# UWQuickstep/quickstep

Measured on AMD Instinct MI355X. Metric: probe+aggregate rows/s at TPC-H SF100 (Q1,Q3), higher is better.
Workload: dtype i32 keys / f64 sums

## Files before the change

quickstep_amd/csrc/join.hip:

```cpp

#include "common.hpp"
#include "join_dense.hpp"
#include "join_lds.hpp"
#include "scan.hpp"

#include <atomic>
#include <cstdlib>
#include <vector>
#include <mutex>
#include <shared_mutex>
#include <type_traits>

namespace qsx {

constexpr int kJBlock = 256;
constexpr uint64_t kEmpty64 = ~0ull;
constexpr uint32_t kEmptyTid = 0xFFFFFFFFu;

struct alignas(16) LongEntry {
  int64_t key;
  uint32_t tid;
  uint32_t pad;
};

constexpr int kBucketSlots = 16;
struct TableView {
  void *slots;
  unsigned char *fp;
  uint64_t buckets;
  unsigned int *dup_flag;
  unsigned int *fill;
  __device__ __host__ uint64_t num_slots() const { return buckets * kBucketSlots; }
};

__device__ __forceinline__ uint64_t home_bucket(int32_t key, const TableView &t) {
  const uint32_t h = static_cast<uint32_t>(key) * 0x9E3779B9u;
  return (static_cast<uint64_t>(h) * t.buckets) >> 32;
}
__device__ __forceinline__ uint32_t fingerprint(int32_t key) {
  const uint32_t f = (static_cast<uint32_t>(key) * 0x85EBCA6Bu) >> 24;
  return f != 0u ? f : 1u;
}
__device__ __forceinline__ uint64_t home_bucket(int64_t key, const TableView &t) {
  const uint64_t h = mix64(static_cast<uint64_t>(key)) * 0x9E3779B97F4A7C15ull;
  return ((h >> 32) * t.buckets) >> 32;
}
__device__ __forceinline__ uint32_t fingerprint(int64_t key) {
  const uint32_t f = static_cast<uint32_t>(mix64(static_cast<uint64_t>(key)) * 0x9E3779B97F4A7C15ull) & 0xFFu;
  return f != 0u ? f : 1u;
}
__device__ __forceinline__ uint32_t zero_bytes(uint32_t x) { return ~(((x & 0x7F7F7F7Fu) + 0x7F7F7F7Fu) | x | 0x7F7F7F7Fu); }
__device__ __forceinline__ uint32_t flags_to_nibble(uint32_t m) { return (((m >> 7) * 0x00204081u) >> 21) & 0xFu; }
__device__ __forceinline__ uint32_t bucket_masks(const uint4 &w, uint32_t f) {
  const uint32_t ffff = f * 0x01010101u;
  const uint32_t same = flags_to_nibble(zero_bytes(w.x ^ ffff)) | flags_to_nibble(zero_bytes(w.y ^ ffff)) << 4 |
                        flags_to_nibble(zero_bytes(w.z ^ ffff)) << 8 | flags_to_nibble(zero_bytes(w.w ^ ffff)) << 12;
  const uint32_t empty = flags_to_nibble(zero_bytes(w.x)) | flags_to_nibble(zero_bytes(w.y)) << 4 | flags_to_nibble(zero_bytes(w.z)) << 8 |
                         flags_to_nibble(zero_bytes(w.w)) << 12;
  return same | empty << 16;
// ... 1424 lines not shown
    (void)qsx_join_table_destroy(shadow);
    shadow = t->shadow = nullptr;
  }
  if (shadow == nullptr) {
    if (qsx_join_table_create_dense(t->key_type, lo, hi, 1, static_cast<int64_t>(entries), &shadow) != QSX_OK) {
      (void)hipGetLastError();
      return stays_hashed();
    }
    t->shadow = shadow;
  } else if (qsx_join_table_clear(shadow, reinterpret_cast<qsx_stream_t>(stream)) != QSX_OK) {
    return stays_hashed();
  }
  shadow->reserved = static_cast<int64_t>(entries);
  shadow->max_tid.store(t->max_tid.load());
  const TableView src = t->view();
  hipLaunchKernelGGL(dense_build_from_slots_kernel, dim3(grid_for(static_cast<int64_t>(src.num_slots()), kJBlock * 4)), dim3(kJBlock), 0, stream,
                     t->key_type == QSX_LONG ? 1 : 0, src, shadow->dense_view());
  if (hipGetLastError() != hipSuccess) return stays_hashed();
  if (seal_verify_enabled()) {
    int error = 0;
    if (hipStreamSynchronize(stream) != hipSuccess ||
        hipMemcpy(&error, shadow->entries_dev + 3, sizeof(error), hipMemcpyDeviceToHost) != hipSuccess || error != 0) {
      set_last_error("QSX_JOIN_SEAL_VERIFY: the shadow's build reported an error", hipErrorUnknown);
      return stays_hashed();
    }
  }
  if (!publish_seal(t, stream, 2)) return stays_hashed();
  return shadow;
}

template <int MODE, bool kRuns, bool kLds = true, int NLIP = 0>
static int launch_lds_dense_probe(qsx_join_table_t *t, const void *keys, int64_t n, int32_t probe_base_tid, const uint64_t *filter,
                                  int32_t *out_probe, int32_t *out_build, int64_t capacity, unsigned long long *count,
                                  uint64_t *out_bitmap, int anti, hipStream_t stream, const long long *runs_dev, int64_t tiles,
                                  const LipViews &lips = LipViews{}) {
  const size_t table_bytes = kLds ? ((static_cast<size_t>(t->range) * 4 + 15) & ~static_cast<size_t>(15)) : 0;
  auto launch = [&](auto key_tag) -> int {
    using KeyT = decltype(key_tag);
    auto kernel = &lds_dense_probe_kernel<KeyT, MODE, kRuns, kLds, NLIP>;
    if (table_bytes > 48 * 1024) {
      QSX_HIP_TRY(hipFuncSetAttribute(reinterpret_cast<const void *>(kernel), hipFuncAttributeMaxDynamicSharedMemorySize, 160 * 1024 - kLdsStaticBytes));
    }
    const int sub = kLds ? kLdsSub : kLdsSubGlobal, per_cu = kLds ? 1 : 2;
    const int64_t units = (tiles + sub - 1) / sub;
    const int grid = static_cast<int>(units < static_cast<int64_t>(per_cu) * kCUs ? units : static_cast<int64_t>(per_cu) * kCUs);
    hipLaunchKernelGGL(kernel, dim3(grid), dim3(kLdsBlock), table_bytes, stream, t->dense_view(), static_cast<const KeyT *>(keys), n, probe_base_tid,
                       filter, out_probe, out_build, capacity, count, out_bitmap, anti, runs_dev, lips);
    QSX_CHECK_LAUNCH();
    return QSX_OK;
  };
  return t->key_type == QSX_INT ? launch(int32_t{}) : launch(int64_t{});
}

static bool one_pass_enabled() {
  const char *e = getenv("QSX_JOIN_ONE_PASS");
  return e == nullptr || e[0] != '0';
}

template <int MODE, bool kRuns = false>
static int launch_probe(qsx_join_table_t *t, const void *keys, int64_t n, int32_t probe_base_tid,
                        const uint64_t *filter, int32_t *out_probe, int32_t *out_build,
                        int64_t capacity, int64_t *out_count, uint64_t *out_bitmap, int anti,
                        hipStream_t stream, const long long *runs_dev = nullptr, int64_t run_tiles = 0) {
  static_assert(kDenseTile == kProbeTile, "one run table serves both table kinds");
  if (!t->dense && n != 0) {
    qsx_join_table *shadow = sealed_shadow(t, stream, n);
    if (shadow != nullptr) {
      return launch_probe<MODE, kRuns>(shadow, keys, n, probe_base_tid, filter, out_probe, out_build, capacity, out_count, out_bitmap,
                                       anti, stream, runs_dev, run_tiles);
    }
    if (!t->scanned.load(std::memory_order_acquire)) {
      set_last_error("the scan in front of a hashed table's first probe could not be issued", hipErrorUnknown);
      return QSX_ERR_HIP;
    }
  }
  const bool zeroed = n != 0 && t->dense && sealed_pack(t, stream, reinterpret_cast<unsigned long long *>(out_count));
  if (out_count != nullptr && !zeroed) QSX_HIP_TRY(hipMemsetAsync(out_count, 0, sizeof(int64_t), stream));
  if (n == 0) return QSX_OK;
  std::shared_lock<std::shared_mutex> lock(t->mutex);
  if (t->dense) {
    const int64_t tiles = kRuns ? run_tiles : (n + kDenseTile - 1) / kDenseTile;
    const int64_t limit = 8 * kCUs;
    const int dgrid = static_cast<int>(tiles < limit ? tiles : limit);
    unsigned long long *dcount = reinterpret_cast<unsigned long long *>(out_count);
    if constexpr (MODE == 0 || MODE == 1 || MODE == 2) {
      const bool two_pass = MODE == 0 && dense_two_pass(filter);
      if (!two_pass && lds_tables_enabled() && t->range <= static_cast<uint64_t>(kLdsDenseMaxWords) && n >= 32 * static_cast<int64_t>(t->range) &&
          n >= (1 << 18)) {
        return launch_lds_dense_probe<MODE, kRuns>(t, keys, n, probe_base_tid, filter, out_probe, out_build, capacity, dcount, out_bitmap, anti,
                                                   stream, runs_dev, tiles);
      }
    }
    if constexpr (MODE == 0) {
      if (dense_two_pass(filter) && one_pass_enabled() && n >= (1 << 20)) {
        return launch_lds_dense_probe<0, kRuns, false>(t, keys, n, probe_base_tid, filter, out_probe, out_build, capacity, dcount, out_bitmap, anti,
                                                       stream, runs_dev, tiles);
      }
    }
    if (MODE == 0 && dense_two_pass(filter)) {
      const int64_t units = tiles * (kDBlock / kWave);
      CallScratch scratch(stream);
      const size_t bytes_counts = static_cast<size_t>(units) * 4, bytes_offsets = static_cast<size_t>(units + 1) * 8,
                   bytes_scan = scan_workspace_words(units) * 8;
      const int rc_scratch = scratch.reserve(CallScratch::padded(bytes_counts) + CallScratch::padded(bytes_offsets) + CallScratch::padded(bytes_scan));
      if (rc_scratch != QSX_OK) return rc_scratch;
      int32_t *unit_counts = static_cast<int32_t *>(scratch.take(bytes_counts));
      int64_t *unit_offsets = static_cast<int64_t *>(scratch.take(bytes_offsets)), *scan_ws = static_cast<int64_t *>(scratch.take(bytes_scan));
      if (t->key_type == QSX_INT) {
        hipLaunchKernelGGL((dense_probe_kernel<int32_t, 3, kRuns>), dim3(dgrid), dim3(kDBlock), 0, stream, t->dense_view(),
                           static_cast<const int32_t *>(keys), n, probe_base_tid, filter, out_probe, out_build, capacity,
                           dcount, out_bitmap, anti, unit_counts, unit_offsets, runs_dev);
      } else {
        hipLaunchKernelGGL((dense_probe_kernel<int64_t, 3, kRuns>), dim3(dgrid), dim3(kDBlock), 0, stream, t->dense_view(),
                           static_cast<const int64_t *>(keys), n, probe_base_tid, filter, out_probe, out_build, capacity,
                           dcount, out_bitmap, anti, unit_counts, unit_offsets, runs_dev);
      }
      QSX_CHECK_LAUNCH();
      QSX_HIP_TRY(launch_scan(unit_counts, units, unit_offsets, out_count, scan_ws, stream));
      if (t->key_type == QSX_INT) {
        hipLaunchKernelGGL((dense_probe_kernel<int32_t, 4, kRuns>), dim3(dgrid), dim3(kDBlock), 0, stream, t->dense_view(),
                           static_cast<const int32_t *>(keys), n, probe_base_tid, filter, out_probe, out_build, capacity,
                           dcount, out_bitmap, anti, unit_counts, unit_offsets, runs_dev);
      } else {
        hipLaunchKernelGGL((dense_probe_kernel<int64_t, 4, kRuns>), dim3(dgrid), dim3(kDBlock), 0, stream, t->dense_view(),
                           static_cast<const int64_t *>(keys), n, probe_base_tid, filter, out_probe, out_build, capacity,
                           dcount, out_bitmap, anti, unit_counts, unit_offsets, runs_dev);
      }
      QSX_CHECK_LAUNCH();
      return QSX_OK;
    }
    if (t->key_type == QSX_INT) {
      hipLaunchKernelGGL((dense_probe_kernel<int32_t, MODE, kRuns>), dim3(dgrid), dim3(kDBlock), 0, stream, t->dense_view(),
                         static_cast<const int32_t *>(keys), n, probe_base_tid, filter, out_probe, out_build, capacity,
                         dcount, out_bitmap, anti, nullptr, nullptr, runs_dev);
    } else {
      hipLaunchKernelGGL((dense_probe_kernel<int64_t, MODE, kRuns>), dim3(dgrid), dim3(kDBlock), 0, stream, t->dense_view(),
                         static_cast<const int64_t *>(keys), n, probe_base_tid, filter, out_probe, out_build, capacity,
                         dcount, out_bitmap, anti, nullptr, nullptr, runs_dev);
    }
    QSX_CHECK_LAUNCH();
    return QSX_OK;
  }
  const int64_t num_tiles = kRuns ? run_tiles : (n + kProbeTile - 1) / kProbeTile;
  if constexpr (MODE == 0 || MODE == 1 || MODE == 2) {
    if (lds_tables_enabled() && t->table_bytes() <= kLdsBucketMaxBytes && n >= (1 << 18) && n >= 8 * static_cast<int64_t>(t->capacity)) {
      const size_t table_bytes = (t->table_bytes() + 15) & ~static_cast<size_t>(15);
      auto launch = [&](auto key_tag) -> int {
        using KeyT = decltype(key_tag);
        auto kernel = &lds_bucket_probe_kernel<KeyT, MODE, kRuns>;
        if (table_bytes > 48 * 1024) {
          QSX_HIP_TRY(hipFuncSetAttribute(reinterpret_cast<const void *>(kernel), hipFuncAttributeMaxDynamicSharedMemorySize, 160 * 1024 - kLdsStaticBytes));
        }
        const int64_t units = (num_tiles + kLdsSub - 1) / kLdsSub;
        const int lgrid = static_cast<int>(units < kCUs ? units : kCUs);
        hipLaunchKernelGGL(kernel, dim3(lgrid), dim3(kLdsBlock), table_bytes, stream, t->view(), static_cast<const KeyT *>(keys), n, probe_base_tid, filter,
                           out_probe, out_build, capacity, reinterpret_cast<unsigned long long *>(out_count), out_bitmap, anti, runs_dev);
        QSX_CHECK_LAUNCH();
        return QSX_OK;
      };
      return t->key_type == QSX_INT ? launch(int32_t{}) : launch(int64_t{});
    }
  }
  const int64_t max_grid = MODE == 0 ? 4 * kCUs : 8 * kCUs;
  const int grid = static_cast<int>(num_tiles < max_grid ? num_tiles : max_grid);
  unsigned long long *count = reinterpret_cast<unsigned long long *>(out_count);
  if constexpr (MODE == 0 || MODE == 1 || MODE == 2) {
    if (t->key_type == QSX_INT && t->seal_state.load(std::memory_order_acquire) == 3 && compact_enabled()) {
      g_compact_probes.fetch_add(1, std::memory_order_relaxed);
      hipLaunchKernelGGL((probe_fp_kernel<int32_t, MODE, kRuns, true>), dim3(grid), dim3(kJBlock), 0, stream, t->view(),
                         static_cast<const int32_t *>(keys), n, probe_base_tid, filter, out_probe,
                         out_build, capacity, count, out_bitmap, anti, runs_dev, t->compact_view());
      QSX_CHECK_LAUNCH();
      return QSX_OK;
    }
  }
  if (t->key_type == QSX_INT) {
    hipLaunchKernelGGL((probe_fp_kernel<int32_t, MODE, kRuns>), dim3(grid), dim3(kJBlock), 0, stream, t->view(),
                       static_cast<const int32_t *>(keys), n, probe_base_tid, filter, out_probe,
                       out_build, capacity, count, out_bitmap, anti, runs_dev);
  } else {
    hipLaunchKernelGGL((probe_fp_kernel<int64_t, MODE, kRuns>), dim3(grid), dim3(kJBlock), 0, stream, t->view(),
                       static_cast<const int64_t *>(keys), n, probe_base_tid, filter, out_probe,
                       out_build, capacity, count, out_bitmap, anti, runs_dev);
  }
  QSX_CHECK_LAUNCH();
  return QSX_OK;
}

static int cover_for(qsx_join_table *t, const ProjectionView &view, int entry_bytes, bool wanted, const std::vector<long long> &signature,
                     hipStream_t stream, const void **cover) {
  const char *env = getenv("QSX_JOIN_COVER");
  if (!wanted || entry_bytes <= 0 || (env != nullptr && env[0] == '0') || !adaptive_enabled()) return 0;
// ... 333 lines not shown
    table[static_cast<size_t>(c)] = proj->width[c];
    table[static_cast<size_t>(nc + c)] = proj->on_build[c] != 0 ? 1 : 0;
    table[static_cast<size_t>(2 * nc + c)] = word_of(proj->out_columns[c]);
    if (proj->on_build[c] != 0) {
      cover_bytes = (cover_bytes + proj->width[c] - 1) / proj->width[c] * proj->width[c];
      table[static_cast<size_t>(3 * nc + c)] = cover_bytes;
      signature.push_back(proj->width[c]);
      signature.push_back(cover_bytes);
      cover_bytes += proj->width[c];
    }
  }
  cover_bytes = cover_bytes == 0 ? 0 : (cover_bytes <= 4 ? 4 : (cover_bytes <= 8 ? 8 : (cover_bytes <= 16 ? 16 : -1)));
  long long seg_rows = 0;
  for (int sg = 0; sg < proj->num_build_segments; ++sg) {
    table[head_words + sg] = proj->build_first_tids[sg];
    signature.push_back(proj->build_first_tids[sg]);
    if (sg > 0) {
      const long long len = proj->build_first_tids[sg] - proj->build_first_tids[sg - 1];
      if (sg == 1) seg_rows = len;
      else if (len != seg_rows) seg_rows = -1;
    }
    for (int c = 0; c < nc; ++c) {
      if (proj->on_build[c] != 0) {
        table[head_words + nseg + static_cast<size_t>(sg) * nc + c] = word_of(proj->build_stripes[static_cast<size_t>(sg) * nc + c]);
        signature.push_back(table[head_words + nseg + static_cast<size_t>(sg) * nc + c]);
      }
    }
  }
  if (seg_rows <= 0 || seg_rows > INT32_MAX) seg_rows = 0;
  const int key_width = direct->key_type == QSX_INT ? 4 : 8;
  for (int c = 0; c < nc; ++c) table[static_cast<size_t>(4 * nc + c)] = proj->on_build[c] == 0 && proj->width[c] == key_width && num_blocks > 0 ? 1 : 0;
  for (int64_t b = 0; b < num_blocks; ++b) {
    for (int c = 0; c < nc; ++c) {
      if (proj->on_build[c] == 0) {
        const void *stripe = proj->probe_stripes[static_cast<size_t>(b) * nc + c];
        if (stripe == nullptr && block_rows[b] > 0) return QSX_ERR_INVALID_ARGUMENT;
        table[head_words + nseg + static_cast<size_t>(nseg) * nc + static_cast<size_t>(b) * nc + c] = word_of(stripe);
        if (block_rows[b] > 0 && stripe != block_keys[b]) table[static_cast<size_t>(4 * nc + c)] = 0;
      }
    }
  }
  const long long *runs_dev = nullptr, *proj_dev = nullptr;
  int64_t tiles = 0, rows = 0;
  bool any_filter = false;
  const int rc = upload_probe_run(num_blocks, block_rows, block_keys, nullptr, block_filters, nullptr, s, &runs_dev, &tiles, &rows,
                                  &any_filter, &table, &proj_dev, coding);
  if (rc != QSX_OK) return rc;
  QSX_HIP_TRY(hipMemsetAsync(out_count_dev, 0, sizeof(int64_t), s));
  if (rows == 0) return QSX_OK;
  sealed_pack(direct, s);
  ProjectionView view{proj_dev, nc, nseg, static_cast<int>(seg_rows), nullptr};
  const int cover_entry = cover_for(direct, view, cover_bytes, any_build && proj->num_build_segments > 0, signature, s, &view.cover);
  std::shared_lock<std::shared_mutex> lock(direct->mutex);
  const int64_t limit = 8 * kCUs;
  const int dgrid = static_cast<int>(tiles < limit ? tiles : limit);
  const uint64_t *filter_mark = any_filter ? reinterpret_cast<const uint64_t *>(runs_dev) : nullptr;
  unsigned long long *count = reinterpret_cast<unsigned long long *>(out_count_dev);
  const DenseTableView dv = direct->dense_view();
  constexpr int kCoverBlock = 512;
  const int cgrid = static_cast<int>(tiles < 4 * kCUs ? tiles : 4 * kCUs);
  auto by_entry = [&](auto key_tag) {
    using KeyT = decltype(key_tag);
    switch (cover_entry) {
      case 4: hipLaunchKernelGGL((cover_probe_kernel<KeyT, uint32_t, kCoverBlock>), dim3(cgrid), dim3(kCoverBlock), 0, s, dv, capacity, count, runs_dev, view); break;
      case 8: hipLaunchKernelGGL((cover_probe_kernel<KeyT, unsigned long long, kCoverBlock>), dim3(cgrid), dim3(kCoverBlock), 0, s, dv, capacity, count, runs_dev, view); break;
      case 16: hipLaunchKernelGGL((cover_probe_kernel<KeyT, ulonglong2, kCoverBlock>), dim3(cgrid), dim3(kCoverBlock), 0, s, dv, capacity, count, runs_dev, view); break;
      default:
        hipLaunchKernelGGL((dense_probe_kernel<KeyT, 5, true>), dim3(dgrid), dim3(kDBlock), 0, s, dv, static_cast<const KeyT *>(nullptr), rows, 0,
                           filter_mark, static_cast<int32_t *>(nullptr), static_cast<int32_t *>(nullptr), capacity, count,
                           static_cast<uint64_t *>(nullptr), 0, static_cast<int32_t *>(nullptr), static_cast<const int64_t *>(nullptr), runs_dev,
                           view);
        break;
    }
  };
  if (direct->key_type == QSX_INT) by_entry(int32_t{}); else by_entry(int64_t{});
  QSX_CHECK_LAUNCH();
  return QSX_OK;
}

static int join_probe_count_blocks_impl(qsx_join_table_t *t, int64_t num_blocks, const int64_t *block_rows, const void *const *block_keys,
                                const uint64_t *const *block_filters, int64_t *out_count_dev, const qsx_key_coding_t *coding, qsx_stream_t stream) {
  QSX_REQUIRE_DEVICE();
  if (t == nullptr || num_blocks < 0 || out_count_dev == nullptr || (num_blocks > 0 && (block_rows == nullptr || block_keys == nullptr))) {
    return QSX_ERR_INVALID_ARGUMENT;
  }
  hipStream_t s = as_stream(stream);
  const long long *runs_dev = nullptr;
  int64_t tiles = 0, rows = 0;
  bool any_filter = false;
  if (check_key_coding(&coding, num_blocks) != QSX_OK) return QSX_ERR_INVALID_ARGUMENT;
  const int rc = upload_probe_run(num_blocks, block_rows, block_keys, nullptr, block_filters, nullptr, s, &runs_dev, &tiles, &rows,
                                  &any_filter, nullptr, nullptr, coding);
  if (rc != QSX_OK) return rc;
  return launch_probe<1, true>(t, nullptr, rows, 0, nullptr, nullptr, nullptr, 0, out_count_dev, nullptr, 0, s, runs_dev, tiles);
}

static int join_probe_exists_blocks_impl(qsx_join_table_t *t, int64_t num_blocks, const int64_t *block_rows, const void *const *block_keys,
                                 const uint64_t *const *block_filters, int anti, uint64_t *const *block_out_bitmaps,
                                 int64_t *out_count_dev, const qsx_key_coding_t *coding, qsx_stream_t stream) {
  QSX_REQUIRE_DEVICE();
  if (t == nullptr || num_blocks < 0 ||
      (num_blocks > 0 && (block_rows == nullptr || block_keys == nullptr || block_out_bitmaps == nullptr))) {
    return QSX_ERR_INVALID_ARGUMENT;
  }
  hipStream_t s = as_stream(stream);
  const long long *runs_dev = nullptr;
  int64_t tiles = 0, rows = 0;
  bool any_filter = false;
  if (check_key_coding(&coding, num_blocks) != QSX_OK) return QSX_ERR_INVALID_ARGUMENT;
  const int rc = upload_probe_run(num_blocks, block_rows, block_keys, nullptr, block_filters, block_out_bitmaps, s, &runs_dev,
                                  &tiles, &rows, &any_filter, nullptr, nullptr, coding);
  if (rc != QSX_OK) return rc;
  return launch_probe<2, true>(t, nullptr, rows, 0, nullptr, nullptr, nullptr, 0, out_count_dev, nullptr, anti, s, runs_dev, tiles);
}

int qsx_join_probe_blocks(qsx_join_table_t *t, int64_t num_blocks, const int64_t *block_rows, const void *const *block_keys,
                          const int32_t *block_base_tids, const uint64_t *const *block_filters, int32_t *out_probe_tid_dev,
                          int32_t *out_build_tid_dev, int64_t capacity, int64_t *out_count_dev, qsx_stream_t stream) {
  return join_probe_blocks_impl(t, num_blocks, block_rows, block_keys, block_base_tids, block_filters, out_probe_tid_dev, out_build_tid_dev,
                                capacity, out_count_dev, nullptr, stream);
}
int qsx_join_probe_blocks_coded(qsx_join_table_t *t, int64_t num_blocks, const int64_t *block_rows, const void *const *block_keys,
                                const qsx_key_coding_t *coding, const int32_t *block_base_tids, const uint64_t *const *block_filters,
                                int32_t *out_probe_tid_dev, int32_t *out_build_tid_dev, int64_t capacity, int64_t *out_count_dev,
// ... 57 lines not shown
```

quickstep_amd/csrc/join_dense.hpp:

```cpp
#ifndef QSX_CSRC_JOIN_DENSE_HPP_
#define QSX_CSRC_JOIN_DENSE_HPP_

#include <type_traits>

#include "block_runs.hpp"
#include "common.hpp"

namespace qsx {

constexpr int kDBlock = 256;
constexpr int kDenseRowsPerThread = 16;
constexpr int kDenseTile = kDBlock * kDenseRowsPerThread;
constexpr uint32_t kChainBit = 0x80000000u;
constexpr int kDenseSparsePairs = 256;

struct DenseTableView {
  uint32_t *head;
  const unsigned char *head3;
  uint2 *ov;
  int64_t min_key;
  int stride_shift;
  uint64_t range;
  unsigned int *ov_count;
  unsigned int ov_capacity;
  int *error;
};

template <typename KeyT>
__device__ __forceinline__ uint64_t dense_index(const DenseTableView &t, KeyT key) {
  const uint64_t d = static_cast<uint64_t>(static_cast<int64_t>(key) - t.min_key);
  const uint64_t idx = d >> t.stride_shift;
  return (idx << t.stride_shift) == d && idx < t.range ? idx : ~0ull;
}

__device__ __forceinline__ uint32_t dense_head_word(const DenseTableView &t, uint64_t idx) {
  if (t.head3 == nullptr) return t.head[idx];
  uint32_t w;
  __builtin_memcpy(&w, t.head3 + idx * 3, 4);
  return (w & 0x7FFFFFu) | ((w & 0x800000u) << 8);
}

__device__ __forceinline__ bool dense_row_in_filter(const uint64_t *filter, int64_t row) {
  return filter == nullptr || ((filter[row >> 6] >> (63 - (row & 63))) & 1u);
}

constexpr int kBuildR = 8;
constexpr int kBuildTile = kBuildR * kWave;
template <typename KeyT, bool kRuns = false>
__global__ __launch_bounds__(kDBlock) void dense_build_kernel(DenseTableView t, const KeyT *__restrict__ keys, int64_t n,
                                                             int32_t base_tid_arg, const uint64_t *__restrict__ filter,
                                                             unsigned long long *__restrict__ entries,
                                                             const long long *__restrict__ runs = nullptr) {
  constexpr int R = kBuildR;
  using Source = ProbeTileSource<KeyT>;
  const int lane = lane_id();
  const int64_t num_groups = kRuns ? runs[2] : (((n + 63) >> 6) + R - 1) / R;
  const int64_t wave = __builtin_amdgcn_readfirstlane(static_cast<int>(blockIdx.x * (kDBlock / kWave) + (threadIdx.x >> 6)));
  const int64_t num_waves = static_cast<int64_t>(gridDim.x) * (kDBlock / kWave);
  unsigned long long inserted = 0;
  KeyT key[R], next_key[R];
  uint64_t words = ~0ull, next_words = ~0ull;
  auto source_of = [&](int64_t group) {
    return probe_tile_source<KeyT, kBuildTile, kRuns>(runs, group, keys, n, base_tid_arg, filter, nullptr);
  };
  auto request = [&](const Source &src, KeyT (&k)[R], uint64_t &fw) {
    const int64_t sw0 = src.base >> 6;
    if (kRuns && src.code_width != 0) {
      coded_keys(src, k, [&](int r) {
        const int64_t row = ((sw0 + r) << 6) + lane;
        return row < src.n ? row : src.n - 1;
      });
    } else {
#pragma unroll
      for (int r = 0; r < R; ++r) {
        const int64_t row = ((sw0 + r) << 6) + lane;
        k[r] = load_global(&src.keys[row < src.n ? row : src.n - 1]);
      }
    }
    fw = ~0ull;
    if (src.filter != nullptr && lane < R && sw0 + lane < ((src.n + 63) >> 6)) fw = load_global(&src.filter[sw0 + lane]);
  };
  Source cur = Source(), next = Source();
  int64_t group = wave;
  if (group < num_groups) {
    cur = source_of(group);
    request(cur, key, words);
  }
  for (; group < num_groups; group += num_waves) {
    if (group + num_waves < num_groups) {
      next = source_of(group + num_waves);
      request(next, next_key, next_words);
    }
// ... 102 lines not shown
    }
    const char *src = p.on_build(c) ? projected_build_value(p, c, width, tid) : p.probe_stripe(tile.block, c) + static_cast<size_t>(probe_row) * width;
    store_value(p.out(c) + o * width, load_value(src, width), width);
  }
}

template <typename EntryT>
__global__ __launch_bounds__(kDBlock) void cover_build_kernel(DenseTableView t, ProjectionView p, EntryT *__restrict__ cover,
                                                             unsigned int *__restrict__ flags) {
  const uint64_t i = static_cast<uint64_t>(blockIdx.x) * kDBlock + threadIdx.x;
  if (i >= t.range) return;
  const uint32_t hw = t.head[i];
  unsigned long long words[2] = {~0ull, ~0ull};
  if (hw & kChainBit) {
    atomicOr(flags, 1u);
  } else if (hw != 0u) {
    words[0] = words[1] = 0ull;
    for (int c = 0; c < p.nc; ++c) {
      if (!p.on_build(c)) continue;
      const int width = p.width(c), off = p.cover_offset(c);
      const unsigned long long v = load_value(projected_build_value(p, c, width, hw - 1u), width);
      if (off < 8) words[0] |= v << (8 * off); else words[1] |= v << (8 * (off - 8));
    }
    const bool ones = sizeof(EntryT) == 4 ? static_cast<uint32_t>(words[0]) == ~0u
                                          : (sizeof(EntryT) == 8 ? words[0] == ~0ull : (words[0] & words[1]) == ~0ull);
    if (ones) atomicOr(flags, 2u);
  }
  if constexpr (sizeof(EntryT) == 4) {
    cover[i] = static_cast<uint32_t>(words[0]);
  } else if constexpr (sizeof(EntryT) == 8) {
    cover[i] = words[0];
  } else {
    cover[i] = EntryT{words[0], words[1]};
  }
}

__device__ __forceinline__ void dense_emit_direct(bool match, int32_t probe_tid, int32_t build_tid,
                                                  int32_t *__restrict__ out_probe, int32_t *__restrict__ out_build,
                                                  unsigned long long capacity, unsigned long long *out_count) {
  const uint64_t m = __ballot(match);
  if (m == 0) return;
  unsigned long long base = 0;
  if (lane_id() == __ffsll(static_cast<long long>(m)) - 1) {
    base = atomicAdd(out_count, static_cast<unsigned long long>(__popcll(m)));
  }
  base = __shfl(base, __ffsll(static_cast<long long>(m)) - 1, kWave);
  const unsigned long long o = base + rank_below(m);
  if (match && o < capacity) {
    __builtin_nontemporal_store(probe_tid, &out_probe[o]);
    __builtin_nontemporal_store(build_tid, &out_build[o]);
  }
}

template <typename KeyT, int MODE, bool kRuns = false>
__global__ __launch_bounds__(kDBlock) __attribute__((amdgpu_waves_per_eu(MODE == 5 ? 3 : 1))) void dense_probe_kernel(
    DenseTableView t, const KeyT *__restrict__ keys, int64_t n, int32_t probe_base_tid,
    const uint64_t *__restrict__ filter, int32_t *__restrict__ out_probe, int32_t *__restrict__ out_build,
    int64_t capacity_signed, unsigned long long *__restrict__ out_count, uint64_t *__restrict__ out_bitmap, int anti,
    int32_t *__restrict__ unit_counts = nullptr, const int64_t *__restrict__ unit_offsets = nullptr,
    const long long *__restrict__ runs = nullptr, ProjectionView proj = ProjectionView{}) {
  constexpr int R = kDenseRowsPerThread;
  constexpr bool kProject = MODE == 5;
  using Source = ProbeTileSource<KeyT>;
  const unsigned long long capacity = static_cast<unsigned long long>(capacity_signed);
  const int64_t num_tiles = kRuns ? runs[2] : (n + kDenseTile - 1) / kDenseTile;
  auto source_of = [&](int64_t tile) {
    return probe_tile_source<KeyT, kDenseTile, kRuns>(runs, tile, keys, n, probe_base_tid, filter, out_bitmap);
  };
  unsigned long long local_count = 0;
  __shared__ int2 s_sparse[(MODE == 0 || MODE == 4) ? kDBlock / kWave : 1][(MODE == 0 || MODE == 4) ? kDenseSparsePairs : 1];
  __shared__ int s_wave_total[2][kDBlock / kWave];
  __shared__ unsigned long long s_tile_base;
  int parity = 0;
  const int wave = threadIdx.x >> 6;

  const int lane = lane_id();
  KeyT key[R], next_key[R];
  uint64_t filter_words = ~0ull, next_filter_words = ~0ull;
  auto request = [&](const Source &src, KeyT (&k)[R], uint64_t &words) {
    if (kRuns && src.code_width != 0) {
      coded_keys(src, k, [&](int r) {
        const int64_t row = src.base + r * kDBlock + threadIdx.x;
        return row < src.n ? row : src.n - 1;
      });
    } else {
#pragma unroll
      for (int r = 0; r < R; ++r) {
        const int64_t row = src.base + r * kDBlock + threadIdx.x;
        k[r] = load_global_nt(&src.keys[row < src.n ? row : src.n - 1]);
      }
    }
    words = ~0ull;
    if (src.filter != nullptr && lane < R) {
      const int64_t w = (src.base >> 6) + lane * (kDBlock / kWave) + wave;
      if (w < ((src.n + 63) >> 6)) words = load_global(&src.filter[w]);
    }
  };
  Source cur = Source(), next = Source();
  if (static_cast<int64_t>(blockIdx.x) < num_tiles) {
    cur = source_of(blockIdx.x);
    request(cur, key, filter_words);
  }

  for (int64_t tile = blockIdx.x; tile < num_tiles; tile += gridDim.x, parity ^= 1) {
    if (tile + gridDim.x < num_tiles) {
      next = source_of(tile + gridDim.x);
      request(next, next_key, next_filter_words);
    }
    const int64_t tile_base = cur.base;
    const int64_t n_rows = cur.n;
    const int32_t base_tid = cur.base_tid;
    uint64_t *const tile_bitmap = cur.out_bitmap;
    const int tile_block = cur.block;
    const Source tile_src = cur;
    cur = next;
    uint32_t h[R];
    uint32_t live_mask = 0;
#pragma unroll
    for (int r = 0; r < R; ++r) {
      const int64_t row = tile_base + r * kDBlock + threadIdx.x;
      const uint64_t filter_word = __shfl(filter_words, r, kWave);
      const bool live = row < n_rows && msb_bit(filter_word, lane);
      live_mask |= live ? (1u << r) : 0u;
      const uint64_t idx = dense_index(t, key[r]);
      const bool lookup = live && idx != ~0ull;
      const uint32_t word = dense_head_word(t, lookup ? idx : 0);
      h[r] = lookup ? word : 0u;
    }
#pragma unroll
    for (int r = 0; r < R; ++r) key[r] = next_key[r];
    filter_words = next_filter_words;

    if (MODE == 2) {
      uint64_t mine = 0;
#pragma unroll
      for (int r = 0; r < R; ++r) {
        const bool bit = ((live_mask >> r) & 1u) && ((h[r] != 0u) != (anti != 0));
        const uint64_t word = msb_first(__ballot(bit));
        if (lane == r) mine = word;
        if (lane == 0) local_count += __popcll(word);
      }
      const int64_t w = (tile_base >> 6) + lane * (kDBlock / kWave) + wave;
      if (lane < R && w < ((n_rows + 63) >> 6)) store_global(mine, &tile_bitmap[w]);
      continue;
    }

    uint64_t m[R];
    int total = 0;
    bool any_chain = false;
#pragma unroll
    for (int r = 0; r < R; ++r) {
      m[r] = __ballot(h[r] != 0u);
      total += __popcll(m[r]);
      any_chain = any_chain || (h[r] & kChainBit) != 0u;
    }
    const bool wave_has_chain = __any(any_chain);
    uint32_t next[R];
    unsigned long long base = 0;
    if (MODE == 1 || MODE == 3) {
      if (lane == 0) local_count += total;
      if (wave_has_chain) {
#pragma unroll
        for (int r = 0; r < R; ++r) next[r] = (h[r] & kChainBit) ? t.ov[h[r] & ~kChainBit].y : 0u;
      }
    } else {
      if (MODE == 0 || kProject) {
        if (lane == 0) s_wave_total[parity][wave] = total;
        __syncthreads();
        if (threadIdx.x == 0) {
          int all = 0;
#pragma unroll
          for (int w = 0; w < kDBlock / kWave; ++w) all += s_wave_total[parity][w];
          s_tile_base = all != 0 ? atomicAdd(out_count, static_cast<unsigned long long>(all)) : 0ull;
        }
        __syncthreads();
        base = s_tile_base;
        for (int w = 0; w < wave; ++w) base += s_wave_total[parity][w];
      } else {
        base = static_cast<unsigned long long>(unit_offsets[tile * (kDBlock / kWave) + wave]);
      }
      const bool sparse = !kProject && total <= kDenseSparsePairs;
      int staged = 0;
      if (kProject) {
        int off[R];
        int emitted = 0;
#pragma unroll
        for (int r = 0; r < R; ++r) {
          next[r] = 0u;
          if (wave_has_chain && (h[r] & kChainBit)) {
            const uint2 e = t.ov[h[r] & ~kChainBit];
            h[r] = e.x + 1u;
            next[r] = e.y;
          }
          off[r] = emitted + rank_below(m[r]);
          emitted += __popcll(m[r]);
        }
        const unsigned long long wave_base = base;
        base += emitted;
        for (int c = 0; c < proj.nc; ++c) {
          const int width = proj.width(c);
          const bool on_build = proj.on_build(c);
          char *dst = proj.out(c);
          const char *probe_stripe = proj.probe_stripe(tile_block, c);
          auto column = [&](auto tag) __attribute__((always_inline)) {
            using V = decltype(tag);
            constexpr int H = R / 2;
#pragma unroll
            for (int half = 0; half < 2; ++half) {
              V v[H];
              if (on_build) {
#pragma unroll
                for (int i = 0; i < H; ++i) {
                  const int r = half * H + i;
                  const char *src = h[r] != 0u ? projected_build_value(proj, c, sizeof(V), h[r] - 1u) : dst;
                  v[i] = load_global(reinterpret_cast<const V *>(src));
                }
              } else if (kRuns && sizeof(V) == sizeof(KeyT) && tile_src.code_width != 0 && proj.is_probe_key(c)) {
#pragma unroll
                for (int i = 0; i < H; ++i) {
                  const int64_t row = tile_base + (half * H + i) * kDBlock + threadIdx.x;
                  v[i] = static_cast<V>(coded_key(tile_src, row < n_rows ? row : n_rows - 1));
                }
              } else {
#pragma unroll
                for (int i = 0; i < H; ++i) {
                  const int64_t row = tile_base + (half * H + i) * kDBlock + threadIdx.x;
                  v[i] = load_global_nt(&reinterpret_cast<const V *>(probe_stripe)[row < n_rows ? row : n_rows - 1]);
                }
              }
#pragma unroll
              for (int i = 0; i < H; ++i) {
                const int r = half * H + i;
                const unsigned long long o = wave_base + off[r];
                if (h[r] != 0u && o < capacity) store_global_nt(v[i], reinterpret_cast<V *>(dst) + o);
              }
            }
          };
          switch (width) {
            case 1: column(uint8_t{}); break;
            case 2: column(uint16_t{}); break;
            case 4: column(uint32_t{}); break;
            default: column(static_cast<unsigned long long>(0)); break;
          }
        }
      }
#pragma unroll
      for (int r = 0; r < R; ++r) {
        if (kProject) break;
        const int64_t row = tile_base + r * kDBlock + threadIdx.x;
        uint32_t tid = h[r] - 1u;
        next[r] = 0u;
        if (wave_has_chain && (h[r] & kChainBit)) {
          const uint2 e = t.ov[h[r] & ~kChainBit];
          tid = e.x;
          next[r] = e.y;
        }
        if (sparse) {
          if (m[r] != 0) {
            if (h[r] != 0u) s_sparse[wave][staged + rank_below(m[r])] = make_int2(static_cast<int32_t>(base_tid + row), static_cast<int32_t>(tid));
            staged += __popcll(m[r]);
          }
        } else {
          const unsigned long long o = base + rank_below(m[r]);
          if (h[r] != 0u && o < capacity) {
            __builtin_nontemporal_store(static_cast<int32_t>(base_tid + row), &out_probe[o]);
            __builtin_nontemporal_store(static_cast<int32_t>(tid), &out_build[o]);
          }
          base += __popcll(m[r]);
        }
      }
      if (sparse) {
        __builtin_amdgcn_fence(__ATOMIC_RELEASE, "wavefront");
        __builtin_amdgcn_wave_barrier();
        __builtin_amdgcn_fence(__ATOMIC_ACQUIRE, "wavefront");
        for (int i = lane; i < total; i += kWave) {
          const int2 pair = s_sparse[wave][i];
          const unsigned long long o = base + i;
          if (o < capacity) {
            __builtin_nontemporal_store(pair.x, &out_probe[o]);
            __builtin_nontemporal_store(pair.y, &out_build[o]);
          }
        }
        base += total;
        __builtin_amdgcn_wave_barrier();
      }
    }
    if (wave_has_chain) {
#pragma unroll 1
      for (int r = 0; r < R; ++r) {
        const int64_t row = tile_base + r * kDBlock + threadIdx.x;
        uint32_t cur = next[r];
        while (__any(cur != 0u)) {
          uint32_t tid = cur - 1u, nxt = 0u;
          if (cur & kChainBit) {
            const uint2 e = t.ov[cur & ~kChainBit];
            tid = e.x;
            nxt = e.y;
          }
          if (MODE == 1 || MODE == 3) {
            local_count += cur != 0u ? 1u : 0u;
          } else if (MODE == 0) {
            dense_emit_direct(cur != 0u, static_cast<int32_t>(base_tid + row), static_cast<int32_t>(tid), out_probe,
                              out_build, capacity, out_count);
          } else if (kProject) {
            const uint64_t cm = __ballot(cur != 0u);
            unsigned long long at = 0;
            const int leader = __ffsll(static_cast<long long>(cm)) - 1;
            if (lane == leader) at = atomicAdd(out_count, static_cast<unsigned long long>(__popcll(cm)));
            at = __shfl(at, leader, kWave) + rank_below(cm);
            if (cur != 0u && at < capacity) project_one(proj, tile_src, row, tid, at);
          } else {
            const uint64_t cm = __ballot(cur != 0u);
            const unsigned long long o = base + rank_below(cm);
            if (cur != 0u && o < capacity) {
              __builtin_nontemporal_store(static_cast<int32_t>(base_tid + row), &out_probe[o]);
              __builtin_nontemporal_store(static_cast<int32_t>(tid), &out_build[o]);
            }
            base += __popcll(cm);
          }
          cur = nxt;
        }
      }
    }
    if (MODE == 3) {
      const unsigned long long unit = wave_reduce_add(local_count);
      if (lane == 0) unit_counts[tile * (kDBlock / kWave) + wave] = static_cast<int32_t>(unit);
      local_count = 0;
    }
  }
  if (MODE == 1 || MODE == 2) {
    local_count = wave_reduce_add(local_count);
    if (lane == 0 && local_count != 0 && out_count != nullptr) atomicAdd(out_count, local_count);
  }
}

template <typename KeyT, typename CoverT, int BLOCK>
__global__ __launch_bounds__(BLOCK) void cover_probe_kernel(DenseTableView t, int64_t capacity_signed,
                                                             unsigned long long *__restrict__ out_count,
                                                             const long long *__restrict__ runs, ProjectionView proj) {
  constexpr int R = kDenseTile / BLOCK;
  static_assert(R * BLOCK == kDenseTile && R <= kWave, "a tile is R steps of BLOCK rows; lane r holds the filter word of step r");
  const unsigned long long capacity = static_cast<unsigned long long>(capacity_signed);
  const int64_t num_tiles = runs[2];
  __shared__ int s_wave_total[2][BLOCK / kWave];
  __shared__ unsigned long long s_tile_base;
  const int wave = threadIdx.x >> 6, lane = lane_id();
  const CoverT *cover = reinterpret_cast<const CoverT *>(proj.cover);
  int parity = 0;
  for (int64_t tile = blockIdx.x; tile < num_tiles; tile += gridDim.x, parity ^= 1) {
    const ProbeTileSource<KeyT> src = probe_tile_source<KeyT, kDenseTile, true>(runs, tile, nullptr, 0, 0, nullptr, nullptr);
    uint64_t filter_words = ~0ull;
    if (src.filter != nullptr && lane < R) {
      const int64_t w = (src.base >> 6) + lane * (BLOCK / kWave) + wave;
      if (w < ((src.n + 63) >> 6)) filter_words = load_global(&src.filter[w]);
    }
    CoverT e[R];
    KeyT key[R];
    {
      if (src.code_width != 0) {
        coded_keys(src, key, [&](int r) {
          const int64_t row = src.base + r * BLOCK + threadIdx.x;
          return row < src.n ? row : src.n - 1;
        });
      } else {
#pragma unroll
        for (int r = 0; r < R; ++r) {
          const int64_t row = src.base + r * BLOCK + threadIdx.x;
          key[r] = load_global_nt(&src.keys[row < src.n ? row : src.n - 1]);
// ... 102 lines not shown
```

Baseline: 195.4 billion.

## Raise dense probe occupancy with 32-bit indexing and occupancy-sized grids

Adds a 32-bit index variant of the dense probe kernel for int keys whose key range fits in 32 bits, and raises the per-kernel waves-per-EU hints. The grid is now sized from the occupancy API instead of a fixed 8 blocks per CU. The kernel also drops the per-row ballot mask array, replaces the filter shuffle with readlane, computes probe tids in 32 bits, and specializes the first-level emit loop on whether chains and sparse staging are present. The goal is lower register pressure so more waves fit on each CU and latency is better hidden. The trade-off is higher waves-per-EU targets that could force spills, plus extra template instantiations.

Measured after the change: 195.5 billion (median of 5 runs). About the same (+0.0%).

```diff
diff --git a/quickstep_amd/csrc/join.hip b/quickstep_amd/csrc/join.hip
--- a/quickstep_amd/csrc/join.hip
+++ b/quickstep_amd/csrc/join.hip
@@ -4,7 +4,10 @@
 #include "join_lds.hpp"
 #include "scan.hpp"
 
+#include <algorithm>
 #include <atomic>
+#include <climits>
+#include <cstdio>
 #include <cstdlib>
 #include <vector>
 #include <mutex>
@@ -1535,6 +1538,51 @@
   return t->key_type == QSX_INT ? launch(int32_t{}) : launch(int64_t{});
 }
 
+template <typename KeyT, int MODE, bool kRuns, bool kIdx32>
+static int dense_probe_resident() {
+  static const int resident = [] {
+    int per_cu = 0;
+    const hipError_t rc = hipOccupancyMaxActiveBlocksPerMultiprocessor(&per_cu, dense_probe_kernel<KeyT, MODE, kRuns, kIdx32>, kDBlock, 0);
+    if (rc != hipSuccess) (void)hipGetLastError();
+    return (rc == hipSuccess && per_cu > 0 ? per_cu : 1) * kCUs;
+  }();
+  return resident;
+}
+static int64_t dense_probe_grid_cap() {
+  const char *e = getenv("QSX_JOIN_DENSE_GRID");
+  return e != nullptr && atoll(e) > 0 ? atoll(e) : INT64_MAX;
+}
+static bool dense_index64_forced() {
+  const char *e = getenv("QSX_JOIN_DENSE_INDEX64");
+  return e != nullptr && e[0] == '1';
+}
+template <int MODE, bool kRuns>
+static void launch_dense_probe_kernel(const qsx_join_table *t, int64_t tiles, hipStream_t stream, const void *keys, int64_t n, int32_t probe_base_tid,
+                                      const uint64_t *filter, int32_t *out_probe, int32_t *out_build, int64_t capacity, unsigned long long *count,
+                                      uint64_t *out_bitmap, int anti, int32_t *unit_counts, const int64_t *unit_offsets, const long long *runs_dev,
+                                      const ProjectionView &proj = ProjectionView{}) {
+  const DenseTableView view = t->dense_view();
+  auto launch = [&](auto key_tag, auto idx32_tag) {
+    using KeyT = decltype(key_tag);
+    constexpr bool kIdx32 = decltype(idx32_tag)::value;
+    const int64_t resident = dense_probe_resident<KeyT, MODE, kRuns, kIdx32>();
+    const int grid = static_cast<int>(std::min(tiles, std::min(resident, dense_probe_grid_cap())));
+    if (getenv("QSX_DEBUG_LAUNCH") != nullptr) {
+      std::fprintf(stderr, "[qsx] dense probe launch mode=%d runs=%d key_bytes=%d idx32=%d grid=%d resident=%lld tiles=%lld\n", MODE, kRuns ? 1 : 0,
+                   static_cast<int>(sizeof(KeyT)), kIdx32 ? 1 : 0, grid, static_cast<long long>(resident), static_cast<long long>(tiles));
+    }
+    hipLaunchKernelGGL((dense_probe_kernel<KeyT, MODE, kRuns, kIdx32>), dim3(grid), dim3(kDBlock), 0, stream, view, static_cast<const KeyT *>(keys), n,
+                       probe_base_tid, filter, out_probe, out_build, capacity, count, out_bitmap, anti, unit_counts, unit_offsets, runs_dev, proj);
+  };
+  if (t->key_type != QSX_INT) {
+    launch(int64_t{}, std::false_type{});
+  } else if (dense_index32_ok(view.min_key, view.stride_shift, view.range) && !dense_index64_forced()) {
+    launch(int32_t{}, std::true_type{});
+  } else {
+    launch(int32_t{}, std::false_type{});
+  }
+}
+
 static bool one_pass_enabled() {
   const char *e = getenv("QSX_JOIN_ONE_PASS");
   return e == nullptr || e[0] != '0';
@@ -1563,8 +1611,6 @@
   std::shared_lock<std::shared_mutex> lock(t->mutex);
   if (t->dense) {
     const int64_t tiles = kRuns ? run_tiles : (n + kDenseTile - 1) / kDenseTile;
-    const int64_t limit = 8 * kCUs;
-    const int dgrid = static_cast<int>(tiles < limit ? tiles : limit);
     unsigned long long *dcount = reinterpret_cast<unsigned long long *>(out_count);
     if constexpr (MODE == 0 || MODE == 1 || MODE == 2) {
       const bool two_pass = MODE == 0 && dense_two_pass(filter);
@@ -1589,38 +1635,17 @@
       if (rc_scratch != QSX_OK) return rc_scratch;
       int32_t *unit_counts = static_cast<int32_t *>(scratch.take(bytes_counts));
       int64_t *unit_offsets = static_cast<int64_t *>(scratch.take(bytes_offsets)), *scan_ws = static_cast<int64_t *>(scratch.take(bytes_scan));
-      if (t->key_type == QSX_INT) {
-        hipLaunchKernelGGL((dense_probe_kernel<int32_t, 3, kRuns>), dim3(dgrid), dim3(kDBlock), 0, stream, t->dense_view(),
-                           static_cast<const int32_t *>(keys), n, probe_base_tid, filter, out_probe, out_build, capacity,
-                           dcount, out_bitmap, anti, unit_counts, unit_offsets, runs_dev);
-      } else {
-        hipLaunchKernelGGL((dense_probe_kernel<int64_t, 3, kRuns>), dim3(dgrid), dim3(kDBlock), 0, stream, t->dense_view(),
-                           static_cast<const int64_t *>(keys), n, probe_base_tid, filter, out_probe, out_build, capacity,
-                           dcount, out_bitmap, anti, unit_counts, unit_offsets, runs_dev);
-      }
+      launch_dense_probe_kernel<3, kRuns>(t, tiles, stream, keys, n, probe_base_tid, filter, out_probe, out_build, capacity, dcount, out_bitmap, anti,
+                                          unit_counts, unit_offsets, runs_dev);
       QSX_CHECK_LAUNCH();
       QSX_HIP_TRY(launch_scan(unit_counts, units, unit_offsets, out_count, scan_ws, stream));
-      if (t->key_type == QSX_INT) {
-        hipLaunchKernelGGL((dense_probe_kernel<int32_t, 4, kRuns>), dim3(dgrid), dim3(kDBlock), 0, stream, t->dense_view(),
-                           static_cast<const int32_t *>(keys), n, probe_base_tid, filter, out_probe, out_build, capacity,
-                           dcount, out_bitmap, anti, unit_counts, unit_offsets, runs_dev);
-      } else {
-        hipLaunchKernelGGL((dense_probe_kernel<int64_t, 4, kRuns>), dim3(dgrid), dim3(kDBlock), 0, stream, t->dense_view(),
-                           static_cast<const int64_t *>(keys), n, probe_base_tid, filter, out_probe, out_build, capacity,
-                           dcount, out_bitmap, anti, unit_counts, unit_offsets, runs_dev);
-      }
+      launch_dense_probe_kernel<4, kRuns>(t, tiles, stream, keys, n, probe_base_tid, filter, out_probe, out_build, capacity, dcount, out_bitmap, anti,
+                                          unit_counts, unit_offsets, runs_dev);
       QSX_CHECK_LAUNCH();
       return QSX_OK;
     }
-    if (t->key_type == QSX_INT) {
-      hipLaunchKernelGGL((dense_probe_kernel<int32_t, MODE, kRuns>), dim3(dgrid), dim3(kDBlock), 0, stream, t->dense_view(),
-                         static_cast<const int32_t *>(keys), n, probe_base_tid, filter, out_probe, out_build, capacity,
-                         dcount, out_bitmap, anti, nullptr, nullptr, runs_dev);
-    } else {
-      hipLaunchKernelGGL((dense_probe_kernel<int64_t, MODE, kRuns>), dim3(dgrid), dim3(kDBlock), 0, stream, t->dense_view(),
-                         static_cast<const int64_t *>(keys), n, probe_base_tid, filter, out_probe, out_build, capacity,
-                         dcount, out_bitmap, anti, nullptr, nullptr, runs_dev);
-    }
+    launch_dense_probe_kernel<MODE, kRuns>(t, tiles, stream, keys, n, probe_base_tid, filter, out_probe, out_build, capacity, dcount, out_bitmap, anti,
+                                           nullptr, nullptr, runs_dev);
     QSX_CHECK_LAUNCH();
     return QSX_OK;
   }
@@ -2060,8 +2085,6 @@
   ProjectionView view{proj_dev, nc, nseg, static_cast<int>(seg_rows), nullptr};
   const int cover_entry = cover_for(direct, view, cover_bytes, any_build && proj->num_build_segments > 0, signature, s, &view.cover);
   std::shared_lock<std::shared_mutex> lock(direct->mutex);
-  const int64_t limit = 8 * kCUs;
-  const int dgrid = static_cast<int>(tiles < limit ? tiles : limit);
   const uint64_t *filter_mark = any_filter ? reinterpret_cast<const uint64_t *>(runs_dev) : nullptr;
   unsigned long long *count = reinterpret_cast<unsigned long long *>(out_count_dev);
   const DenseTableView dv = direct->dense_view();
@@ -2074,10 +2097,8 @@
       case 8: hipLaunchKernelGGL((cover_probe_kernel<KeyT, unsigned long long, kCoverBlock>), dim3(cgrid), dim3(kCoverBlock), 0, s, dv, capacity, count, runs_dev, view); break;
       case 16: hipLaunchKernelGGL((cover_probe_kernel<KeyT, ulonglong2, kCoverBlock>), dim3(cgrid), dim3(kCoverBlock), 0, s, dv, capacity, count, runs_dev, view); break;
       default:
-        hipLaunchKernelGGL((dense_probe_kernel<KeyT, 5, true>), dim3(dgrid), dim3(kDBlock), 0, s, dv, static_cast<const KeyT *>(nullptr), rows, 0,
-                           filter_mark, static_cast<int32_t *>(nullptr), static_cast<int32_t *>(nullptr), capacity, count,
-                           static_cast<uint64_t *>(nullptr), 0, static_cast<int32_t *>(nullptr), static_cast<const int64_t *>(nullptr), runs_dev,
-                           view);
+        launch_dense_probe_kernel<5, true>(direct, tiles, s, nullptr, rows, 0, filter_mark, nullptr, nullptr, capacity, count, nullptr, 0, nullptr, nullptr,
+                                           runs_dev, view);
         break;
     }
   };
diff --git a/quickstep_amd/csrc/join_dense.hpp b/quickstep_amd/csrc/join_dense.hpp
--- a/quickstep_amd/csrc/join_dense.hpp
+++ b/quickstep_amd/csrc/join_dense.hpp
@@ -12,6 +12,12 @@
 constexpr int kDenseRowsPerThread = 16;
 constexpr int kDenseTile = kDBlock * kDenseRowsPerThread;
 constexpr uint32_t kChainBit = 0x80000000u;
+constexpr int dense_probe_min_waves(int key_bytes, int mode, bool runs, bool idx32) {
+  if (mode == 5) return 3;
+  if (runs) return 1;
+  if (key_bytes == 8) return 4;
+  return idx32 && mode != 0 && mode != 4 ? 6 : 5;
+}
 constexpr int kDenseSparsePairs = 256;
 
 struct DenseTableView {
@@ -33,11 +39,42 @@
   return (idx << t.stride_shift) == d && idx < t.range ? idx : ~0ull;
 }
 
+__device__ __forceinline__ uint64_t lane_word(uint64_t v, int src) {
+  const uint32_t lo = static_cast<uint32_t>(__builtin_amdgcn_readlane(static_cast<int>(static_cast<uint32_t>(v)), src));
+  const uint32_t hi = static_cast<uint32_t>(__builtin_amdgcn_readlane(static_cast<int>(static_cast<uint32_t>(v >> 32)), src));
+  return (static_cast<uint64_t>(hi) << 32) | lo;
+}
+
 __device__ __forceinline__ uint32_t dense_head_word(const DenseTableView &t, uint64_t idx) {
   if (t.head3 == nullptr) return t.head[idx];
   uint32_t w;
   __builtin_memcpy(&w, t.head3 + idx * 3, 4);
   return (w & 0x7FFFFFu) | ((w & 0x800000u) << 8);
+}
+
+__device__ __forceinline__ uint32_t dense_index32(const DenseTableView &t, int32_t key) {
+  const uint32_t d = static_cast<uint32_t>(key) - static_cast<uint32_t>(t.min_key);
+  const uint32_t idx = d >> t.stride_shift;
+  return (idx << t.stride_shift) == d && idx < static_cast<uint32_t>(t.range) ? idx : ~0u;
+}
+struct DenseHeadWords {
+  const unsigned char *base;
+  uint32_t wide;
+  uint32_t value_mask;
+  uint32_t chain_mask;
+  __device__ __forceinline__ explicit DenseHeadWords(const DenseTableView &t)
+      : base(t.head3 != nullptr ? t.head3 : reinterpret_cast<const unsigned char *>(t.head)), wide(t.head3 != nullptr ? 0u : 1u),
+        value_mask(t.head3 != nullptr ? 0x7FFFFFu : 0xFFFFFFFFu), chain_mask(t.head3 != nullptr ? 0x800000u : 0u) {}
+  template <typename IdxT>
+  __device__ __forceinline__ uint32_t word(IdxT idx) const {
+    uint32_t w;
+    __builtin_memcpy(&w, base + ((idx << 1) + (idx << wide)), 4);
+    return (w & value_mask) | ((w & chain_mask) << 8);
+  }
+};
+inline bool dense_index32_ok(int64_t min_key, int stride_shift, uint64_t range) {
+  if (range == 0 || range > (1ull << 30) || stride_shift > 31 || min_key < INT32_MIN || min_key > INT32_MAX) return false;
+  return min_key + static_cast<int64_t>((range - 1) << stride_shift) <= INT32_MAX;
 }
 
 __device__ __forceinline__ bool dense_row_in_filter(const uint64_t *filter, int64_t row) {
@@ -246,8 +283,8 @@
   }
 }
 
-template <typename KeyT, int MODE, bool kRuns = false>
-__global__ __launch_bounds__(kDBlock) __attribute__((amdgpu_waves_per_eu(MODE == 5 ? 3 : 1))) void dense_probe_kernel(
+template <typename KeyT, int MODE, bool kRuns = false, bool kIdx32 = false>
+__global__ __launch_bounds__(kDBlock) __attribute__((amdgpu_waves_per_eu(dense_probe_min_waves(sizeof(KeyT), MODE, kRuns, kIdx32)))) void dense_probe_kernel(
     DenseTableView t, const KeyT *__restrict__ keys, int64_t n, int32_t probe_base_tid,
     const uint64_t *__restrict__ filter, int32_t *__restrict__ out_probe, int32_t *__restrict__ out_build,
     int64_t capacity_signed, unsigned long long *__restrict__ out_count, uint64_t *__restrict__ out_bitmap, int anti,
@@ -295,6 +332,7 @@
     cur = source_of(blockIdx.x);
     request(cur, key, filter_words);
   }
+  const DenseHeadWords heads(t);
 
   for (int64_t tile = blockIdx.x; tile < num_tiles; tile += gridDim.x, parity ^= 1) {
     if (tile + gridDim.x < num_tiles) {
@@ -308,18 +346,25 @@
     const int tile_block = cur.block;
     const Source tile_src = cur;
     cur = next;
+    const int tile_rows = static_cast<int>(n_rows - tile_base < kDenseTile ? n_rows - tile_base : kDenseTile);
+    const uint32_t tile_tid = static_cast<uint32_t>(base_tid) + static_cast<uint32_t>(tile_base);
     uint32_t h[R];
     uint32_t live_mask = 0;
 #pragma unroll
     for (int r = 0; r < R; ++r) {
-      const int64_t row = tile_base + r * kDBlock + threadIdx.x;
-      const uint64_t filter_word = __shfl(filter_words, r, kWave);
-      const bool live = row < n_rows && msb_bit(filter_word, lane);
+      const bool live = r * kDBlock + static_cast<int>(threadIdx.x) < tile_rows && msb_bit(lane_word(filter_words, r), lane);
       live_mask |= live ? (1u << r) : 0u;
-      const uint64_t idx = dense_index(t, key[r]);
-      const bool lookup = live && idx != ~0ull;
-      const uint32_t word = dense_head_word(t, lookup ? idx : 0);
-      h[r] = lookup ? word : 0u;
+      if constexpr (kIdx32) {
+        const uint32_t idx = dense_index32(t, key[r]);
+        const bool lookup = live && idx != ~0u;
+        const uint32_t word = heads.word(lookup ? idx : 0u);
+        h[r] = lookup ? word : 0u;
+      } else {
+        const uint64_t idx = dense_index(t, key[r]);
+        const bool lookup = live && idx != ~0ull;
+        const uint32_t word = heads.word(lookup ? idx : 0ull);
+        h[r] = lookup ? word : 0u;
+      }
     }
 #pragma unroll
     for (int r = 0; r < R; ++r) key[r] = next_key[r];
@@ -339,24 +384,18 @@
       continue;
     }
 
-    uint64_t m[R];
     int total = 0;
-    bool any_chain = false;
+    uint32_t chain_bits = 0u;
 #pragma unroll
     for (int r = 0; r < R; ++r) {
-      m[r] = __ballot(h[r] != 0u);
-      total += __popcll(m[r]);
-      any_chain = any_chain || (h[r] & kChainBit) != 0u;
-    }
-    const bool wave_has_chain = __any(any_chain);
-    uint32_t next[R];
+      total += __popcll(__ballot(h[r] != 0u));
+      chain_bits |= h[r];
+    }
+    const bool wave_has_chain = __any((chain_bits & kChainBit) != 0u);
+    uint32_t next[kProject ? R : 1];
     unsigned long long base = 0;
     if (MODE == 1 || MODE == 3) {
       if (lane == 0) local_count += total;
-      if (wave_has_chain) {
-#pragma unroll
-        for (int r = 0; r < R; ++r) next[r] = (h[r] & kChainBit) ? t.ov[h[r] & ~kChainBit].y : 0u;
-      }
     } else {
       if (MODE == 0 || kProject) {
         if (lane == 0) s_wave_total[parity][wave] = total;
@@ -386,8 +425,9 @@
             h[r] = e.x + 1u;
             next[r] = e.y;
           }
-          off[r] = emitted + rank_below(m[r]);
-          emitted += __popcll(m[r]);
+          const uint64_t m = __ballot(h[r] != 0u);
+          off[r] = emitted + rank_below(m);
+          emitted += __popcll(m);
         }
         const unsigned long long wave_base = base;
         base += emitted;
@@ -438,29 +478,34 @@
           }
         }
       }
-#pragma unroll
-      for (int r = 0; r < R; ++r) {
-        if (kProject) break;
-        const int64_t row = tile_base + r * kDBlock + threadIdx.x;
-        uint32_t tid = h[r] - 1u;
-        next[r] = 0u;
-        if (wave_has_chain && (h[r] & kChainBit)) {
-          const uint2 e = t.ov[h[r] & ~kChainBit];
-          tid = e.x;
-          next[r] = e.y;
-        }
-        if (sparse) {
-          if (m[r] != 0) {
-            if (h[r] != 0u) s_sparse[wave][staged + rank_below(m[r])] = make_int2(static_cast<int32_t>(base_tid + row), static_cast<int32_t>(tid));
-            staged += __popcll(m[r]);
+      auto first_level = [&](auto chains_tag, auto sparse_tag) __attribute__((always_inline)) {
+        constexpr bool kChains = decltype(chains_tag)::value, kSparse = decltype(sparse_tag)::value;
+#pragma unroll
+        for (int r = 0; r < R; ++r) {
+          uint32_t tid = h[r] - 1u;
+          if (kChains && (h[r] & kChainBit)) tid = t.ov[h[r] & ~kChainBit].x;
+          const int32_t probe_tid = static_cast<int32_t>(tile_tid + static_cast<uint32_t>(r * kDBlock) + threadIdx.x);
+          const uint64_t m = __ballot(h[r] != 0u);
+          if (kSparse) {
+            if (m != 0) {
+              if (h[r] != 0u) s_sparse[wave][staged + rank_below(m)] = make_int2(probe_tid, static_cast<int32_t>(tid));
+              staged += __popcll(m);
+            }
+          } else {
+            const unsigned long long o = base + rank_below(m);
+            if (h[r] != 0u && o < capacity) {
+              __builtin_nontemporal_store(probe_tid, &out_probe[o]);
+              __builtin_nontemporal_store(static_cast<int32_t>(tid), &out_build[o]);
+            }
+            base += __popcll(m);
           }
+        }
+      };
+      if constexpr (!kProject) {
+        if (wave_has_chain) {
+          if (sparse) first_level(std::true_type{}, std::true_type{}); else first_level(std::true_type{}, std::false_type{});
         } else {
-          const unsigned long long o = base + rank_below(m[r]);
-          if (h[r] != 0u && o < capacity) {
-            __builtin_nontemporal_store(static_cast<int32_t>(base_tid + row), &out_probe[o]);
-            __builtin_nontemporal_store(static_cast<int32_t>(tid), &out_build[o]);
-          }
-          base += __popcll(m[r]);
+          if (sparse) first_level(std::false_type{}, std::true_type{}); else first_level(std::false_type{}, std::false_type{});
         }
       }
       if (sparse) {
@@ -483,7 +528,13 @@
 #pragma unroll 1
       for (int r = 0; r < R; ++r) {
         const int64_t row = tile_base + r * kDBlock + threadIdx.x;
-        uint32_t cur = next[r];
+        const int32_t probe_tid = static_cast<int32_t>(tile_tid + static_cast<uint32_t>(r * kDBlock) + threadIdx.x);
+        uint32_t cur;
+        if constexpr (kProject) {
+          cur = next[r];
+        } else {
+          cur = (h[r] & kChainBit) ? t.ov[h[r] & ~kChainBit].y : 0u;
+        }
         while (__any(cur != 0u)) {
           uint32_t tid = cur - 1u, nxt = 0u;
           if (cur & kChainBit) {
@@ -494,7 +545,7 @@
           if (MODE == 1 || MODE == 3) {
             local_count += cur != 0u ? 1u : 0u;
           } else if (MODE == 0) {
-            dense_emit_direct(cur != 0u, static_cast<int32_t>(base_tid + row), static_cast<int32_t>(tid), out_probe,
+            dense_emit_direct(cur != 0u, probe_tid, static_cast<int32_t>(tid), out_probe,
                               out_build, capacity, out_count);
           } else if (kProject) {
             const uint64_t cm = __ballot(cur != 0u);
@@ -507,7 +558,7 @@
             const uint64_t cm = __ballot(cur != 0u);
             const unsigned long long o = base + rank_below(cm);
             if (cur != 0u && o < capacity) {
-              __builtin_nontemporal_store(static_cast<int32_t>(base_tid + row), &out_probe[o]);
+              __builtin_nontemporal_store(probe_tid, &out_probe[o]);
               __builtin_nontemporal_store(static_cast<int32_t>(tid), &out_build[o]);
             }
             base += __popcll(cm);
```
